# steinwurf/storage-benchmarks

Measured on AMD Instinct MI355X. Metric: encode+decode goodput GiB/s (device-resident) at symbols x symbol_size; %HBM roofline, higher is better.
Workload: dtype u8; 1 GPU; isa_throughput c3: symbols=64 symbol_size=1000000 loss_rate=0.5 erased=32 blocks_per_gpu=1024; symbols=64, symbol_size=1000000, erased=32, parallelism=blocks sharded x1, no collective, decode_kernel=auto, encode_kernel=auto

## Files before the change

storage-benchmarks_amd/csrc/jit_prog.cpp:

```cpp
#include "jit_prog.h"

#include <string.h>

#include <algorithm>

#include "rs_jit.h"
#include "rs_kernels.h"

namespace rsgpu {
namespace jit {

namespace {

inline int value_reg(int v, int bank) { return v < 8 ? plane_reg(bank, v) : 32 + (v - 8); }

void full_tables(const uint8_t (&masks)[8 * kMaxSlots], int nm, SrcProg& p)
{
    uint8_t id[256];
    memset(id, kNone, sizeof id);
    for (int a = 0; a < 8; ++a)
        id[1 << a] = (uint8_t)a;
    p.nops = 0;
    for (int hi = 0; hi < 2; ++hi)
        for (int n = 1; n < 16; ++n) {
// ... 505 lines not shown
            for (int b = 0; b < 8; ++b)
                acc[b] = 40 + 8 * r + b;
            if (!emit_scale_add(w, role == 1 ? 1 : kp.sigma[r], 10, 18, acc))
                return 0;
        }
        w.put64(ret);
        return w.o;
    }
    const uint8_t* m = role == 0 ? kp.cP : role == 1 ? kp.cQ1 : kp.cQ2;
    for (int i = 0; i < kKaraPairs; ++i) {
        const int s = kKaraPairs * ch + i;
        if (role == 0) {
            emit_load_planes(w, 10, 2 * i);
            emit_load_planes(w, 18, 2 * i + 1);
            w.put32(enc_waitcnt_lgkm(0));
            const int pl[8] = {10, 11, 12, 13, 14, 15, 16, 17};
            if (!emit_scale_add(w, kp.rho[s], 18, 26, pl))
                return 0;
        } else {
            emit_load_planes(w, 10, 2 * i + (role - 1));
            w.put32(enc_waitcnt_lgkm(0));
        }
        uint8_t cf[16];
        for (int r = 0; r < 16; ++r)
            cf[r] = m[r * 32 + s];
        SrcProg prog;
        plan_source(cf, 16, prog);
        emit_source_body(w, 16, prog);
    }
    w.put64(ret);
    return w.o;
}

}

bool build_karatsuba_code(const uint8_t* c, KaraProgram* out)
{
    KaraProgram& kp = *out;
    auto c2 = [](int n) { return n * (n - 1) / 2; };
    auto h = [&](int n) { return gf_pow2(c2(n)); };
    uint8_t d[64], D1[32];
    for (int j = 0; j < 64; ++j)
        d[j] = gf_pow2(-c2(j));
    for (int r = 0; r < 32; ++r)
        D1[r] = gf_pow2(-c2(r));
    for (int r = 0; r < 16; ++r)
        kp.sigma[r] = gf_mul(D1[r + 16], gf_inv(D1[r]));
    for (int base = 0; base < 64; base += 32)
        for (int q = 0; q < 16; ++q) {
            const int s = 16 * (base / 32) + q;
            kp.rho[s] = gf_mul(d[base + 16 + q], gf_inv(d[base + q]));
            for (int r = 0; r < 16; ++r) {
                const uint8_t hb = h(r + q + base + 16);
                kp.cP[r * 32 + s] = gf_mul(gf_mul(D1[r], hb), d[base + q]);
                kp.cQ1[r * 32 + s] = gf_mul(gf_mul(D1[r], (uint8_t)(h(r + q + base) ^ hb)), d[base + q]);
                kp.cQ2[r * 32 + s] =
                    gf_mul(gf_mul(D1[r + 16], (uint8_t)(h(r + q + base + 32) ^ hb)), d[base + 16 + q]);
                const uint8_t p = kp.cP[r * 32 + s], pr = gf_mul(p, kp.rho[s]);
                if ((uint8_t)(p ^ kp.cQ1[r * 32 + s]) != c[r * 64 + base + q] || pr != c[r * 64 + base + 16 + q] ||
                    gf_mul(kp.sigma[r], p) != c[(16 + r) * 64 + base + q] ||
                    (uint8_t)(gf_mul(kp.sigma[r], pr) ^ kp.cQ2[r * 32 + s]) != c[(16 + r) * 64 + base + 16 + q])
                    return false;
            }
        }
    size_t most = 0;
    for (int role = 0; role < 3; ++role)
        for (int ch = 0; ch < kKaraChunks; ++ch) {
            const size_t n = emit_chunk_kara(nullptr, kp, role, ch);
            if (!n)
                return false;
            most = std::max(most, n);
        }
    kp.chunk_stride = (int)((most + 63) / 64 * 64);
    kp.code.assign((size_t)3 * kKaraChunks * kp.chunk_stride, 0);
    for (size_t i = 0; i + 8 <= kp.code.size(); i += 8) {
        const uint64_t ret = (uint64_t)S_NOP0 << 32 | S_SETPC_82;
        memcpy(&kp.code[i], &ret, 8);
    }
    for (int role = 0; role < 3; ++role)
        for (int ch = 0; ch < kKaraChunks; ++ch)
            emit_chunk_kara(&kp.code[((size_t)role * kKaraChunks + ch) * kp.chunk_stride], kp, role, ch);
    return true;
}

}
}
```

storage-benchmarks_amd/csrc/jit_prog.h:

```cpp
#pragma once
#include <stddef.h>
#include <stdint.h>

#include <utility>
#include <vector>

namespace rsgpu {
namespace jit {

constexpr int kMaxComposites = 22;
constexpr uint8_t kNone = 255;

constexpr int kMaxSlots = 16;

struct SrcProg {
    int nops = 0;
    uint8_t ops[kMaxComposites][3];
    uint8_t outs[8 * kMaxSlots][2];
};

void plan_source(const uint8_t* coef, int nslot, SrcProg& p, int max_ops = kMaxComposites);

int host_chunk_stride();

size_t emit_chunk(uint8_t* dst, int nt, int nslot, const SrcProg* progs);

std::vector<uint8_t> build_matrix_code(const uint8_t* c, int k, int e, int* chunk_stride,
                                       int max_ops = kMaxComposites);

std::vector<uint8_t> build_matrix_code_wide(const uint8_t* c, int k, int e, int R, int CS, int* chunk_stride,
                                            int max_ops = kMaxComposites);

std::vector<uint8_t> build_matrix_code_wide_passes(const uint8_t* c, int k, int e,
                                                   std::vector<std::pair<size_t, int>>* passes,
                                                   int max_ops = kMaxComposites);

struct KaraProgram {
    std::vector<uint8_t> code;
    int chunk_stride = 0;
    uint8_t cP[16 * 32], cQ1[16 * 32], cQ2[16 * 32];
    uint8_t rho[32], sigma[16];
};

bool build_karatsuba_code(const uint8_t* c, KaraProgram* out);

}
}
```

storage-benchmarks_amd/csrc/rs_jit.h:

```cpp
#pragma once
#include <stdint.h>

#include "jit_enc.h"
#include "kernel_hooks.h"

namespace rsgpu {
namespace jit {

constexpr int ACC = 64;
constexpr int PRO_BYTES = 16;
constexpr int PRE_BYTES = 112;
constexpr int EPI_BYTES = 8;

RJ_HD constexpr int src_bytes(int nslot) { return PRE_BYTES + 64 * nslot; }
RJ_HD constexpr int chunk_bytes(int nt, int nslot) { return PRO_BYTES + nt * src_bytes(nslot) + EPI_BYTES; }
RJ_HD constexpr int chunk_stride(int nslot) { return (chunk_bytes(8, nslot) + 63) / 64 * 64; }

RJ_HD constexpr int plane_reg(int bank, int a) { return (bank ? 54 : 24) + a; }

RJ_HD constexpr int table_reg(int bank, int hi, int n)
{
    if ((n & (n - 1)) == 0) {
        const int a = n == 1 ? 0 : n == 2 ? 1 : n == 4 ? 2 : 3;
        return plane_reg(bank, 4 * hi + a);
// ... 138 lines not shown
        const int low = n & -n;
        return enc_xor_e32(treg(hi, n), treg(hi, n ^ low), treg(hi, low));
    }

    RJ_HD static bool code_word(const uint8_t* rows, int k, int nslot, int ch, int o, uint64_t* word)
    {
        const int nt = k - CS * ch < CS ? k - CS * ch : CS;
        const int per_src = PRE / 8 + 8 * nslot;
        if (o < nt * per_src) {
            const int t = o / per_src, r = o - t * per_src;
            if (r < PRE / 8) {
                *word = (uint64_t)pre_u32(t, 2 * r + 1) << 32 | pre_u32(t, 2 * r);
            } else {
                const int m = r - PRE / 8, s = m >> 3;
                uint64_t wd[8];
                mac_words(rows[s * k + CS * ch + t], s, wd);
                *word = wd[m & 7];
            }
        } else if (o == nt * per_src) {
            *word = (uint64_t)S_NOP0 << 32 | S_SETPC_82;
        } else {
            return false;
        }
        return true;
    }
};
using J16 = Wide<16, 6>;
using J12 = Wide<12, 6>;
using J10 = Wide<10, 5>;

constexpr int kKaraPairs = 4;
constexpr int kKaraSrcChunks = 32 / kKaraPairs;
constexpr int kKaraChunks = kKaraSrcChunks + 1;
RJ_HD constexpr int kara_source(int ch, int t)
{
    const int s = kKaraPairs * ch + t / 2;
    return 32 * (s / 16) + (s % 16) + 16 * (t & 1);
}

struct WideTables {
    static constexpr int PW = Wide<16, 6>::PRE / 8;
    uint64_t mac[256 * 8];
    uint64_t pre[6 * PW];
};
RJ_HD constexpr WideTables wide_tables()
{
    WideTables w{};
    for (int c = 0; c < 256; ++c)
        for (int b = 0; b < 8; ++b)
            w.mac[8 * c + b] = J16::mac_base(mat_row((uint8_t)c, b));
    for (int t = 0; t < 6; ++t)
        for (int r = 0; r < WideTables::PW; ++r)
            w.pre[WideTables::PW * t + r] = (uint64_t)J16::pre_u32(t, 2 * r + 1) << 32 | J16::pre_u32(t, 2 * r);
    return w;
}

}
}
```

storage-benchmarks_amd/csrc/rs_jit.hip:

```cpp
#include <hip/hip_runtime.h>
#include <stdint.h>

#include <algorithm>
#include <cstring>
#include <type_traits>
#include <utility>

#include "bitslice.h"
#include "diag_clock.h"
#include "rs_jit.h"
#include "rs_kernels.h"
#include "rs_lane.h"
#include "rs_span.h"
#include "tc_handlers.inc"

namespace rsgpu {
namespace jitk {

using bs::barrier_lds;
using bs::glds32;
using bs::glds32_nt;
using bs::sload_ptr;
using bs::store32;
using bs::tr8;
// ... 741 lines not shown
                         : RSGPU_JW_CALL_CLOBBERS, "s82", "s83", "scc", "memory", RSGPU_J12_ACC_CLOBBERS);
        else
            asm volatile("s_swappc_b64 s[82:83], %[fn]"
                         :
                         : [fn] "s"(fn), "{v9}"(la)
                         : RSGPU_JW_CALL_CLOBBERS, "s82", "s83", "scc", "memory", RSGPU_J10_ACC_CLOBBERS);
        ph.mark(5);
    }
    epi.template run<W, TPW, NV>(a, dsts, bw, wave, tw, lane, off, &lds[0][0][0]);
    ph.mark(6);
    ph.end(wv);
}

template <class W, int TPW, int NV>
__global__ __launch_bounds__(64 * NV * TPW) __attribute__((amdgpu_num_vgpr(40))) void k_rs_jitw(JitArgs a)
{
    __shared__ uint4 lds[2][TPW][W::CS * 2 * 64];
    RSGPU_DIAG_BEGIN()
    const int wv = __builtin_amdgcn_readfirstlane(threadIdx.x >> 6);
    const int wave = wv % NV, tw = wv / NV;
    const int lane = threadIdx.x & 63;
    RSGPU_JIT_PLACE(a, b, wg)
    const long long tile = wg * TPW + tw;
    if (a.status && a.status[b] != 0)
        return;
    jitw_run<W, TPW, NV>(a, lds, wv, wave, tw, lane, b, wg, tile, JitwStore{});
    RSGPU_DIAG_END();
}

__global__ __launch_bounds__(64 * 3) __attribute__((amdgpu_num_vgpr(40))) void k_rs_kara(JitArgs a)
{
    constexpr int CS = 2 * jit::kKaraPairs, NCH = jit::kKaraSrcChunks, K = 64;
    __shared__ uint4 lds[2][CS * 2 * 64];
    const int role = __builtin_amdgcn_readfirstlane(threadIdx.x >> 6);
    const int lane = threadIdx.x & 63;
    RSGPU_JIT_PLACE(a, b, tile)
    const uint8_t* const* srcs = a.srcs + (size_t)b * K;
    uint8_t* const* dsts = a.dsts + (size_t)b * a.dst_stride;
    const uint8_t* code = a.code + (size_t)role * jit::kKaraChunks * a.chunk_stride;
    const uint32_t lds0 = (uint32_t)(uintptr_t)(__attribute__((address_space(3))) uint4*)&lds[0][0];
    constexpr uint32_t kBuf = CS * 2 * 64 * 16;
    const long long off = tile * 2048 + lane * 32;
    const uint32_t loff = off + 32 <= a.len ? (uint32_t)off : 0u;
    if (role == 0)
        asm volatile("s_icache_inv\n s_nop 15\n s_nop 15" ::: "memory");
    typedef const uint8_t* const __attribute__((address_space(4)))* CPtrs;
    const CPtrs csrcs = (CPtrs)srcs;
    const int first = role == 0 ? 2 : role - 1;
    constexpr int PW = 3;
    auto ptrs = [&](int ch, const uint8_t* (&p)[PW]) {
#pragma unroll
        for (int i = 0; i < PW; ++i)
            p[i] = csrcs[jit::kara_source(ch, min(first + 3 * i, CS - 1))];
    };
    auto issue = [&](int par, const uint8_t* const (&p)[PW]) {
        const uint32_t base = lds0 + (uint32_t)(par * kBuf);
#pragma unroll
        for (int i = 0; i < PW; ++i) {
            const int t = first + 3 * i;
            if (t < CS)
                glds32(p[i], loff, base + (uint32_t)(t * 2 * 64 * 16));
        }
    };
    asm volatile(RSGPU_J16_ZERO ::: RSGPU_J16_ACC_CLOBBERS);
    int rot = 0;
    if (a.chunk_rot_ticks > 0) {
        volatile int& s_rot = *(volatile int*)&lds[1][0];
        if (threadIdx.x == 0) {
            unsigned long long t;
            asm volatile("s_memrealtime %0\n s_waitcnt lgkmcnt(0)" : "=s"(t)::"memory");
            const unsigned long long p = (unsigned long long)a.chunk_rot_ticks;
            s_rot = (int)(((t + p / 2) / p) % (unsigned long long)NCH);
        }
        __syncthreads();
        rot = __builtin_amdgcn_readfirstlane(s_rot);
    }
    auto chunk_of = [&](int i) { return i + rot >= NCH ? i + rot - NCH : i + rot; };
    const uint8_t* pc[PW];
    const uint8_t* pn[PW];
    ptrs(chunk_of(0), pc);
    issue(0, pc);
    ptrs(chunk_of(1), pn);
    for (int i = 0; i < NCH; ++i) {
        const int ch = chunk_of(i), par = i & 1;
        uint4* buf = lds[par];
        wait_vm(0);
        if (a.prio)
            asm volatile("s_setprio 2" ::: "memory");
        {
            const uint32_t m4 = vconst(0x0F0F0F0Fu), m2 = vconst(0x33333333u), m1 = vconst(0x55555555u);
            for (int t = first; t < CS; t += 3) {
                uint4 u = buf[(t * 2 + 0) * 64 + lane], v = buf[(t * 2 + 1) * 64 + lane];
                uint32_t Wd[8] = {u.x, u.y, u.z, u.w, v.x, v.y, v.z, v.w};
                tr8(Wd, m4, m2, m1);
                buf[(t * 2 + 0) * 64 + lane] = make_uint4(Wd[0], Wd[1], Wd[2], Wd[3]);
                buf[(t * 2 + 1) * 64 + lane] = make_uint4(Wd[4], Wd[5], Wd[6], Wd[7]);
            }
        }
        barrier_lds();
        if (a.prio)
            asm volatile("s_setprio 0" ::: "memory");
        if (i + 1 < NCH)
            issue(par ^ 1, pn);
        ptrs(chunk_of(min(i + 2, NCH - 1)), pn);
        const uint32_t la = lds0 + (uint32_t)(par * kBuf) + lane * 16;
        const uint8_t* fn = code + (size_t)ch * a.chunk_stride;
        asm volatile("s_swappc_b64 s[82:83], %[fn]"
                     :
                     : [fn] "s"(fn), "{v9}"(la)
                     : RSGPU_JW_CALL_CLOBBERS, "s82", "s83", "scc", "memory", RSGPU_J16_ACC_CLOBBERS);
    }
    barrier_lds();
    if (role == 0) {
        uint4* tb = &lds[0][0];
        [&]<int... Ss>(std::integer_sequence<int, Ss...>) {
            (
                [&] {
                    uint32_t Wd[8];
                    read_slotw<Ss>(Wd);
                    tb[(Ss * 2 + 0) * 64 + lane] = make_uint4(Wd[0], Wd[1], Wd[2], Wd[3]);
                    tb[(Ss * 2 + 1) * 64 + lane] = make_uint4(Wd[4], Wd[5], Wd[6], Wd[7]);
                }(),
                ...);
        }(std::make_integer_sequence<int, 16>{});
    }
    barrier_lds();
    if (role != 0) {
        const uint32_t la = lds0 + lane * 16;
        const uint8_t* fn = code + (size_t)NCH * a.chunk_stride;
        asm volatile("s_swappc_b64 s[82:83], %[fn]"
                     :
                     : [fn] "s"(fn), "{v9}"(la)
                     : RSGPU_JW_CALL_CLOBBERS, "s82", "s83", "scc", "memory", RSGPU_J16_ACC_CLOBBERS);
        const int half = role - 1;
        JitwStore{}.run<jit::J16, 1, 2>(a, dsts, b, half, 0, lane, off, nullptr);
    }
}

template <class W, int TPW, int NV>
__global__ __launch_bounds__(64 * NV * TPW) __attribute__((amdgpu_num_vgpr(40))) void k_rs_jitw_scrub(JitScrubArgs s)
{
    __shared__ uint4 lds[2][TPW][W::CS * 2 * 64];
    const int wv = __builtin_amdgcn_readfirstlane(threadIdx.x >> 6);
    const int wave = wv % NV, tw = wv / NV;
    const int lane = threadIdx.x & 63;
    RSGPU_JIT_PLACE(s.j, b, wg)
    const long long tile = wg * TPW + tw;
    jitw_run<W, TPW, NV>(s.j, lds, wv, wave, tw, lane, b, wg, tile, JitwScrub{{s.fold, s.tab, s.locate}});
}

template <class W, int TPW, int NV>
__global__ __launch_bounds__(64 * NV * TPW) __attribute__((amdgpu_num_vgpr(40))) void k_rs_jitw_locate(JitLocateArgs s)
{
    __shared__ uint4 lds[2][TPW][W::CS * 2 * 64];
    const int wv = __builtin_amdgcn_readfirstlane(threadIdx.x >> 6);
    const int wave = wv % NV, tw = wv / NV;
    const int lane = threadIdx.x & 63;
    RSGPU_JIT_PLACE(s.j, b, wg)
    const long long tile = wg * TPW + tw;
    jitw_run<W, TPW, NV>(s.j, lds, wv, wave, tw, lane, b, wg, tile,
                         JitwLocate{{s.fold, s.cand, s.cand_stride, s.slots, s.u}});
}

template <class W, int TPW, int NV>
__global__ __launch_bounds__(64 * NV * TPW) __attribute__((amdgpu_num_vgpr(40))) void k_rs_jitw_repair(JitRepairArgs s)
{
    __shared__ uint4 lds[2][TPW][W::CS * 2 * 64];
    const int wv = __builtin_amdgcn_readfirstlane(threadIdx.x >> 6);
    const int wave = wv % NV, tw = wv / NV;
// ... 420 lines not shown
```

storage-benchmarks_amd/csrc/rs_kernels.h:

```cpp
#pragma once
#include <hip/hip_runtime.h>
#include <stdint.h>

struct rsgpu_scrub_report;

namespace rsgpu {

constexpr size_t kMaxGridBlocks = 65535;

struct DotArgs {
    const uint8_t* const* srcs;
    uint8_t* const* dsts;
    const uint4* tabs4;
    const uint32_t* ctab;
    long long tab_block_stride;
    int k, rows, rows_pad;
    long long len;
    long long blocks;
    const int* status;
    bool bytewise;
};

struct PrepArgs {
    int k, m, nerrs, rows_pad;
// ... 82 lines not shown
    long long pitch, len, blocks;
    int k, e;
    const uint8_t* rowtab;
    const uint8_t* coef;
    RepairFold* fold;
    int mode;
};
hipError_t launch_repair_compare(const RepairCmpArgs& a, hipStream_t st);
hipError_t launch_repair_finalise(void* report, long long blocks, int mode, hipStream_t st);
hipError_t launch_rs_bitsliced_repair(int k, int e, uint8_t* src, uint8_t* par, long long pitch, long long len,
                                      long long blocks, RepairFold* fold, int mode, hipStream_t st);

hipError_t launch_decode_prepare_syn(int k, int e, long long blocks, const uint8_t* err,
                                     uint8_t* out, long long out_pitch, const uint8_t** srcs,
                                     uint8_t** dsts, const unsigned long long* tc_table, int* status,
                                     const uint8_t* src, const uint8_t* par,
                                     unsigned long long* dir_addr, uint8_t* jit_coef, hipStream_t st);

struct JitArgs {
    const uint8_t* const* srcs;
    uint8_t* const* dsts;
    const uint8_t* code;
    long long chunk_stride;
    long long block_stride;
    int k, rows;
    int dst_stride;
    long long len;
    const int* status;
    int xcd_order;
    int tiles_per_wg = 1;
    int code_prefetch = 0;
    int chunk_rot_ticks = 0;
    int prio = 0;
};
int jitw_rot_ticks(int rows);
size_t jit_code_bytes(int k, int e, long long blocks);
hipError_t launch_jit_emit(int k, int e, long long blocks, const uint8_t* coef, const int* status,
                           uint8_t* code, hipStream_t st);
hipError_t launch_jit_fill(void* code, size_t bytes, hipStream_t st);
hipError_t launch_rs_jit(const JitArgs& a, long long blocks, hipStream_t st);
int jitw_rows(int e);
int jitw_cs(int e);
size_t jitw_chunk_stride(int e);
size_t jitw_code_bytes(int k, int e, long long blocks);
bool jitw_layout(int e);
size_t jitw_pass_bytes(int k, int rows);
size_t jitw_pass_offset(int k, int e, int p);
hipError_t launch_jitw_emit(int k, int e, long long blocks, const uint8_t* coef, const int* status,
                            uint8_t* code, hipStream_t st);
hipError_t launch_rs_jitw(const JitArgs& a, long long blocks, hipStream_t st);
hipError_t launch_rs_kara(const JitArgs& a, long long blocks, hipStream_t st);
struct JitScrubArgs {
    JitArgs j;
    ScrubFold* fold;
    const uint8_t* tab;
    int locate;
};
hipError_t launch_rs_jit_scrub(const JitScrubArgs& a, long long blocks, hipStream_t st);
struct JitLocateArgs {
    JitArgs j;
    ScrubFold* fold;
    uint8_t* cand;
    size_t cand_stride;
    int slots;
    int u;
};
// ... 207 lines not shown
```

storage-benchmarks_amd/csrc/rsgpu_capi.cpp:

```cpp
#include <hip/hip_runtime.h>
#include <hsa/hsa.h>
#include <hsa/hsa_ext_amd.h>

#include <algorithm>
#include <climits>
#include <cstdio>
#include <cstdlib>
#include <cstring>
#include <string>
#include <vector>

#include "../../include/rsgpu.h"
#include "gf256.h"
#include "rsgpu_ctx.h"
#include "rsgpu_internal.h"
#include "jit_prog.h"
#include "rs_jit.h"
#include "rs_kernels.h"
#include "rs_synth.h"

namespace {

using namespace rsgpu;

// ... 47 lines not shown
    hsa_amd_memory_pool_get_info(p, HSA_AMD_MEMORY_POOL_INFO_RUNTIME_ALLOC_ALLOWED, &alloc);
    if ((flags & HSA_AMD_MEMORY_POOL_GLOBAL_FLAG_COARSE_GRAINED) && alloc) {
        *(hsa_amd_memory_pool_t*)out = p;
        return HSA_STATUS_INFO_BREAK;
    }
    return HSA_STATUS_SUCCESS;
}

constexpr size_t kProgCacheEntries = 64;
constexpr size_t kProgCacheBytes = 256u << 20;

const rsgpu_ctx::SharedProg* shared_program(rsgpu_ctx* ctx, const uint8_t* coef, int k, int rows, int* rc_out,
                                            bool kara = false)
{
    *rc_out = RSGPU_OK;
    const bool wide = jitw_layout(rows);
    std::vector<uint8_t> key(9 + (size_t)k * rows);
    std::memcpy(key.data(), &k, 4);
    std::memcpy(key.data() + 4, &rows, 4);
    key[8] = kara ? 2 : wide ? 1 : 0;
    std::memcpy(key.data() + 9, coef, (size_t)k * rows);
    for (auto& pr : ctx->progs)
        if (pr.key == key) {
            pr.last = ++ctx->prog_tick;
            return &pr;
        }
    auto err = [&](int code, const char* msg) -> const rsgpu_ctx::SharedProg* {
        *rc_out = fail(ctx, code, msg);
        return nullptr;
    };
    if (jit_probe(ctx) != 1)
        return err(RSGPU_ERR_UNSUPPORTED, "no executable device memory pool");
    int stride = 0;
    std::vector<uint8_t> code;
    std::vector<std::pair<size_t, int>> passes;
    if (kara) {
        jit::KaraProgram kp;
        if (k != 64 || rows != 32 || !jit::build_karatsuba_code(coef, &kp))
            return err(RSGPU_ERR_UNSUPPORTED, "Karatsuba program: not the (64, 32) gf_gen_rs_matrix code");
        code = std::move(kp.code);
        stride = kp.chunk_stride;
    } else if (wide) {
        code = jit::build_matrix_code_wide_passes(coef, k, rows, &passes);
        if (code.empty())
            return err(RSGPU_ERR_UNSUPPORTED, "shared program: rows exceed the layout");
    } else {
        code = jit::build_matrix_code(coef, k, rows, &stride);
    }
    size_t used = 0;
    for (const auto& pr : ctx->progs)
        used += pr.bytes;
    if (!ctx->progs.empty() &&
        (ctx->progs.size() >= kProgCacheEntries || used + code.size() > kProgCacheBytes)) {
        if (hipStreamSynchronize(ctx->stream) != hipSuccess)
            return err(RSGPU_ERR_HIP, "shared program: draining the stream before an eviction");
        while (!ctx->progs.empty() &&
               (ctx->progs.size() >= kProgCacheEntries || used + code.size() > kProgCacheBytes)) {
            auto lru = std::min_element(ctx->progs.begin(), ctx->progs.end(),
                                        [](const auto& a, const auto& b) { return a.last < b.last; });
            used -= lru->bytes;
            hsa_amd_memory_pool_free(lru->code);
            ctx->progs.erase(lru);
        }
    }
    if (ctx->code_stage_bytes < code.size()) {
        if (hipStreamSynchronize(ctx->stream) != hipSuccess)
            return err(RSGPU_ERR_HIP, "shared program: draining the stream before regrowing the stage");
        if (ctx->d_code_stage)
            (void)hipFree(ctx->d_code_stage);
        ctx->d_code_stage = nullptr;
        ctx->code_stage_bytes = 0;
        if (hipMalloc(&ctx->d_code_stage, code.size()) != hipSuccess)
            return err(RSGPU_ERR_NOMEM, "shared program: code stage allocation failed");
        ctx->code_stage_bytes = code.size();
    }
    rsgpu_ctx::SharedProg pr;
    if (hsa_amd_memory_pool_allocate(ctx->jit_pool, code.size(), HSA_AMD_MEMORY_POOL_EXECUTABLE_FLAG,
                                     &pr.code) != HSA_STATUS_SUCCESS || !pr.code)
        return err(RSGPU_ERR_NOMEM, "executable device allocation failed");
    pr.bytes = code.size();
    void* stage;
    int rc = get_stage(ctx, code.size(), &stage);
    if (!rc) {
        std::memcpy(stage, code.data(), code.size());
        rc = upload(ctx, ctx->d_code_stage, code.size());
    }
    if (!rc && launch_jit_copy(pr.code, ctx->d_code_stage, code.size(), ctx->stream) != hipSuccess)
        rc = fail(ctx, RSGPU_ERR_HIP, "shared program: copy into executable memory");
    if (rc) {
        hsa_amd_memory_pool_free(pr.code);
        *rc_out = rc;
        return nullptr;
    }
    pr.key = std::move(key);
    pr.chunk_stride = stride;
    pr.passes = std::move(passes);
    pr.last = ++ctx->prog_tick;
    ctx->progs.push_back(std::move(pr));
    return &ctx->progs.back();
}

JitArgs shared_pass_args(const rsgpu_ctx* ctx, const rsgpu_ctx::SharedProg* pg, int k, int rows, int p,
                         long long len, const uint8_t* const* d_srcs, uint8_t* const* d_dsts)
{
    if (jitw_layout(rows)) {
        JitArgs j = jit_args(d_srcs, d_dsts + jit::wide_pass_row0(rows, p),
                             (const uint8_t*)pg->code + pg->passes[p].first, pg->passes[p].second, 0, k,
                             jit::wide_pass_rows(rows, p), rows, len, nullptr);
        j.tiles_per_wg = ctx->jitw_tpw ? ctx->jitw_tpw : 2;
        j.chunk_rot_ticks = ctx->jitw_rot >= 0 ? ctx->jitw_rot : jitw_rot_ticks(j.rows);
        j.prio = ctx->jitw_prio;
        return j;
    }
    const int nch = (k + 7) / 8;
    JitArgs j = jit_args(d_srcs, d_dsts + 32 * p, (const uint8_t*)pg->code + (size_t)p * 4 * nch * pg->chunk_stride,
                         pg->chunk_stride, 0, k, std::min(32, rows - 32 * p), rows, len, nullptr);
    j.prio = 0;
    return j;
}

int shared_program_launch(rsgpu_ctx* ctx, const uint8_t* coef, int k, int rows, long long len,
                          long long blocks, const uint8_t* const* d_srcs, uint8_t* const* d_dsts,
                          const char* name)
{
    int rc = RSGPU_OK;
    const rsgpu_ctx::SharedProg* pg = shared_program(ctx, coef, k, rows, &rc);
    if (!pg)
        return rc;
    const bool wide = jitw_layout(rows);
    for (int p = 0; wide ? p < jit::wide_passes(rows) : p * 32 < rows; ++p) {
// ... 98 lines not shown
size_t dot_table_bytes(int k, int rows)
{
    return std::max(sizeof(unsigned long long) * (size_t)tc_table_elems(k, rows),
                    (size_t)k * rows_pad_for(rows) * (sizeof(uint4) + sizeof(uint32_t)));
}

constexpr long long kKaraMinWork = 480000;
constexpr int kKaraRotTicks = 400;

int karatsuba_launch(rsgpu_ctx* ctx, long long len, size_t pitch, size_t blocks, const unsigned char* d_src,
                     unsigned char* d_parity, bool* unavailable)
{
    const int k = 64, e = 32;
    *unavailable = false;
    const std::vector<uint8_t> c = parity_matrix(k, e, nullptr);
    int rc = RSGPU_OK;
    const std::string err_before = ctx->err;
    const rsgpu_ctx::SharedProg* pg = shared_program(ctx, c.data(), k, e, &rc, true);
    if (!pg && rc == RSGPU_ERR_UNSUPPORTED) {
        ctx->kara_state = -1;
        ctx->err = err_before;
        *unavailable = true;
        return RSGPU_OK;
    }
    if (!pg)
        return rc;
    RowPtrs rp;
    rc = row_ptr_tables(ctx, k, e, pitch, blocks, d_src, d_parity, rp);
    if (rc)
        return rc;
    JitArgs j = jit_args(rp.src, rp.par, pg->code, pg->chunk_stride, 0, k, e, e, len, nullptr);
    j.chunk_rot_ticks = ctx->jitw_rot >= 0 ? ctx->jitw_rot : kKaraRotTicks;
    j.prio = ctx->jitw_prio;
    KTimer kt(ctx, "k_rs_jit(encode)", blocks);
    RS_HIP(ctx, launch_rs_kara(j, (long long)blocks, ctx->stream));
    return RSGPU_OK;
}

int encode_slice(rsgpu_ctx* ctx, int k, int e, size_t len, size_t pitch, size_t blocks, const unsigned char* d_src,
                 unsigned char* d_parity, const unsigned char* coef)
{
    const bool aligned = ptrs_aligned(pitch, d_src, d_parity);
    const bool kara_wanted = ctx->encode_kernel == RSGPU_ENCODE_KARATSUBA ||
                             (ctx->encode_kernel == RSGPU_ENCODE_AUTO &&
                              (long long)(tiles(len) * blocks) >=
                                  (ctx->kara_min_work >= 0 ? ctx->kara_min_work : kKaraMinWork));
    if (kara_wanted && ctx->kara_state >= 0 && !coef && k == 64 && e == 32 && aligned && len % 32 == 0 &&
        jit_probe(ctx) == 1) {
        bool unavailable;
        const int rc = karatsuba_launch(ctx, (long long)len, pitch, blocks, d_src, d_parity, &unavailable);
        if (!unavailable)
            return rc;
    }
    const bool compiled_ok = ctx->encode_kernel == RSGPU_ENCODE_AUTO || ctx->encode_kernel == RSGPU_ENCODE_COMPILED ||
                             ctx->encode_kernel == RSGPU_ENCODE_KARATSUBA;
    if (compiled_ok && !coef && aligned && len % 32 == 0 && rs_bitsliced_split_available(k, e) &&
        (long long)(tiles(len) * blocks) < kTcSplitMaxWork) {
        KTimer kt(ctx, "k_rs_bs_split(encode)", blocks);
        RS_HIP(ctx, launch_rs_bitsliced_split(k, e, d_src, d_parity, (long long)pitch, (long long)len,
                                              (long long)blocks, ctx->stream));
        return RSGPU_OK;
    }
    const bool compiled_pays = ctx->encode_kernel == RSGPU_ENCODE_COMPILED ||
                               rs_bitsliced_rows_per_wave(k, e) >= 8 || !jitw_rows(e) ||
                               !(len % 32 == 0 && jit_probe(ctx) == 1);
    if (compiled_ok && compiled_pays && !coef && aligned && len % 32 == 0 && rs_bitsliced_available(k, e)) {
// ... 255 lines not shown
    return RSGPU_OK;
}

int rsgpu_destroy(rsgpu_ctx* ctx)
{
    if (!ctx)
        return RSGPU_ERR_ARG;
    (void)hipSetDevice(ctx->device);
    (void)hipStreamSynchronize(ctx->stream);
    for (void* p : {ctx->scratch.p, ctx->scrub.p, ctx->d_update, ctx->degraded.p, ctx->rebuild.p,
                    ctx->locate.p})
        if (p)
            (void)hipFree(p);
    if (ctx->h_stage)
        (void)hipHostFree(ctx->h_stage);
    if (ctx->stage_done)
        (void)hipEventDestroy(ctx->stage_done);
    for (auto& r : ctx->recs) {
        (void)hipEventDestroy(r.a);
        (void)hipEventDestroy(r.b);
    }
    for (auto e : ctx->ev_pool)
        (void)hipEventDestroy(e);
    for (auto e : ctx->sync_evs)
        (void)hipEventDestroy(e);
    if (ctx->d_tc_table)
        (void)hipFree(ctx->d_tc_table);
    if (ctx->d_jit)
        hsa_amd_memory_pool_free(ctx->d_jit);
    for (auto& pr : ctx->progs)
        hsa_amd_memory_pool_free(pr.code);
    if (ctx->d_code_stage)
        (void)hipFree(ctx->d_code_stage);
    for (hipStream_t st : {ctx->io_in, ctx->io_out, ctx->aux})
        if (st) {
            (void)hipStreamSynchronize(st);
            (void)hipStreamDestroy(st);
        }
    if (ctx->d_io)
        (void)hipFree(ctx->d_io);
    for (auto e : ctx->io_evs)
        (void)hipEventDestroy(e);
    delete ctx;
    return RSGPU_OK;
}

int rsgpu_set_stream(rsgpu_ctx* ctx, void* s)
{
    if (!ctx)
        return RSGPU_ERR_ARG;
    hipStream_t ns = (hipStream_t)s;
    if (ns == ctx->stream)
        return RSGPU_OK;
    hipEvent_t ev = sync_event(ctx);
    hipError_t e = hipEventRecord(ev, ctx->stream);
    if (e == hipSuccess)
        e = hipStreamWaitEvent(ns, ev, 0);
    ctx->stream = ns;
    if (e != hipSuccess)
        return fail(ctx, RSGPU_ERR_HIP, std::string("rsgpu_set_stream: ordering against the old stream: ") +
                                            hipGetErrorString(e));
    return RSGPU_OK;
}

void* rsgpu_get_stream(rsgpu_ctx* ctx) { return ctx ? (void*)ctx->stream : nullptr; }

// ... 316 lines not shown
```

storage-benchmarks_amd/csrc/rsgpu_ctx.h:

```cpp
#pragma once
#include <hip/hip_runtime.h>
#include <hsa/hsa.h>
#include <hsa/hsa_ext_amd.h>

#include <string>
#include <vector>

#include "../../include/rsgpu.h"

struct rsgpu_ctx {
    int device = 0;
    hipStream_t stream = nullptr;
    std::vector<hipEvent_t> sync_evs;
    size_t sync_next = 0;
    unsigned long long* d_tc_table = nullptr;
    unsigned long long h_tc_table[2048] = {};
    unsigned long long tc_base = 0;
    int tc_state = 0;
    int decode_kernel = RSGPU_DECODE_AUTO;
    int jitw_tpw = 0;
    long long kara_min_work = -1;
    int kara_state = 0;
    int jitw_prefetch = -1;
    int jitw_rot = -1;
    int bs_prio = 2;
    int jitw_prio = 2;
    int decode_pipe = -1;
    hipStream_t aux = nullptr;
    void* d_jit = nullptr;
    size_t jit_bytes = 0;
    int jit_state = 0;
    unsigned long long jit_gen = 0;
    struct {
        int k = 0, e = 0;
        size_t blocks = 0;
        const void* ws = nullptr;
        unsigned long long gen = 0;
    } jit_key;
    hsa_amd_memory_pool_t jit_pool{};
    int encode_kernel = RSGPU_ENCODE_AUTO;
    struct SharedProg {
        std::vector<uint8_t> key;
        void* code = nullptr;
        size_t bytes = 0;
        int chunk_stride = 0;
        std::vector<std::pair<size_t, int>> passes;
        unsigned long long last = 0;
    };
    std::vector<SharedProg> progs;
    unsigned long long prog_tick = 0;
    void* d_code_stage = nullptr;
    size_t code_stage_bytes = 0;
    std::string err;
    struct DevBuf {
        void* p = nullptr;
        size_t bytes = 0;
        std::vector<uint8_t> key;
    };
    DevBuf scratch;
    int scrub_kernel = RSGPU_SCRUB_AUTO;
    DevBuf scrub;
    void* d_update = nullptr;
    std::vector<uint8_t> update_key;
    DevBuf degraded;
    int degraded_kernel = RSGPU_DEGRADED_AUTO;
    int correct_kernel = RSGPU_CORRECT_AUTO;
    int repair_kernel = RSGPU_REPAIR_KERNEL_AUTO;
    DevBuf rebuild;
    int rebuild_kernel = RSGPU_REBUILD_AUTO;
    struct RebuildWideLayout {
        size_t blocks = 0, lane = 0, lane_stride = 0, addr = 0, srcs = 0, dsts = 0, count = 0;
        int k = 0, passes = 0, slots = 0;
    } rebuild_wide;
    size_t rebuild_group_max = 0;
    bool rebuild_prepare_only = false;
    int locate_kernel = RSGPU_LOCATE_AUTO;
    DevBuf locate;
    size_t locate_group_max = 0;
    void* h_stage = nullptr;
    size_t stage_bytes = 0;
    hipEvent_t stage_done = nullptr;
    bool stage_pending = false;
    bool timing = false;
// ... 47 lines not shown
```

storage-benchmarks_amd/csrc/rsgpu_testhooks.cpp:

```cpp
#include <hip/hip_runtime.h>

#include <algorithm>
#include <cstdint>
#include <cstring>
#include <vector>

#include "../../include/rsgpu.h"
#include "jit_prog.h"
#include "plane_mul.h"
#include "rs_jit.h"
#include "rs_kernels.h"
#include "rs_lane.h"
#include "rs_pairs.h"
#include "rsgpu_ctx.h"

using namespace rsgpu;

namespace {

template <class W>
void jitw_emit_host(int k, int row_base, int rows, const unsigned char* coef, uint64_t* o64)
{
    const int nch = (k + W::CS - 1) / W::CS, stride_w = W::chunk_stride() / 8;
    for (int w = 0; w < jit::wide_waves(rows); ++w) {
// ... 185 lines not shown
                                          size_t out_bytes, long long* pass_off, int* pass_stride, int max_passes,
                                          int* npasses, int max_ops)
{
    if (k <= 0 || k + e > 250 || !jitw_layout(e) || !coef || !pass_off || !pass_stride || !npasses)
        return -1;
    std::vector<std::pair<size_t, int>> passes;
    const std::vector<uint8_t> code = jit::build_matrix_code_wide_passes(coef, k, e, &passes, max_ops);
    if (code.empty() || (int)passes.size() > max_passes)
        return -1;
    *npasses = (int)passes.size();
    for (size_t p = 0; p < passes.size(); ++p) {
        pass_off[p] = (long long)passes[p].first;
        pass_stride[p] = passes[p].second;
    }
    if (out && out_bytes >= code.size())
        std::memcpy(out, code.data(), code.size());
    return (long long)code.size();
}

long long rsgpu_internal_jit_karatsuba_code(const unsigned char* coef, unsigned char* out, size_t out_bytes,
                                            int* chunk_stride, unsigned char* mats)
{
    jit::KaraProgram kp;
    if (!coef || !chunk_stride || !jit::build_karatsuba_code(coef, &kp))
        return -1;
    *chunk_stride = kp.chunk_stride;
    if (mats) {
        std::memcpy(mats, kp.cP, 512);
        std::memcpy(mats + 512, kp.cQ1, 512);
        std::memcpy(mats + 1024, kp.cQ2, 512);
        std::memcpy(mats + 1536, kp.rho, 32);
        std::memcpy(mats + 1568, kp.sigma, 16);
    }
    if (out && out_bytes >= kp.code.size())
        std::memcpy(out, kp.code.data(), kp.code.size());
    return (long long)kp.code.size();
}

int rsgpu_internal_set_kara_min_work(rsgpu_ctx* ctx, long long pairs)
{
    if (!ctx || pairs < -1)
        return RSGPU_ERR_ARG;
    ctx->kara_min_work = pairs;
    return RSGPU_OK;
}

int rsgpu_internal_set_kara_state(rsgpu_ctx* ctx, int state)
{
    if (!ctx || (state != 0 && state != -1))
        return RSGPU_ERR_ARG;
    ctx->kara_state = state;
    return RSGPU_OK;
}

long long rsgpu_internal_jitw_emit_device(rsgpu_ctx* ctx, int k, int e, size_t blocks,
                                          const unsigned char* coef, unsigned char* out, size_t out_bytes)
{
    if (!ctx || k <= 0 || !jitw_layout(e) || k + e > 250 || blocks == 0 || blocks > kMaxGridBlocks || !coef)
        return -1;
    const size_t need = jitw_code_bytes(k, e, (long long)blocks);
    if (!out || out_bytes < need)
        return (long long)need;
    uint8_t *d_coef = nullptr, *d_code = nullptr;
    int* d_status = nullptr;
    long long rc = -1;
    if (hipMalloc(&d_coef, blocks * e * k) == hipSuccess && hipMalloc(&d_code, need) == hipSuccess &&
        hipMalloc(&d_status, blocks * sizeof(int)) == hipSuccess &&
        hipMemcpyAsync(d_coef, coef, blocks * e * k, hipMemcpyHostToDevice, ctx->stream) == hipSuccess &&
        hipMemsetAsync(d_status, 0, blocks * sizeof(int), ctx->stream) == hipSuccess &&
        launch_jit_fill(d_code, need, ctx->stream) == hipSuccess &&
        launch_jitw_emit(k, e, (long long)blocks, d_coef, d_status, d_code, ctx->stream) == hipSuccess &&
        hipMemcpyAsync(out, d_code, need, hipMemcpyDeviceToHost, ctx->stream) == hipSuccess &&
        hipStreamSynchronize(ctx->stream) == hipSuccess)
        rc = (long long)need;
    (void)hipFree(d_coef);
    (void)hipFree(d_code);
// ... 68 lines not shown
```

Baseline: 1443 GiB/s.

## Split Karatsuba epilogue across three waves and gate icache invalidation by generation

The Karatsuba encode kernel's final combine step, previously done by two waves while wave 0 only staged slots, is now split so all three waves run JIT-emitted epilogue chunks and each stores part of the parity rows directly. Separately, the per-launch s_icache_inv is replaced by a per-CU generation table, so the cache is invalidated only when a newer code upload is seen. This aims to balance epilogue work across waves and to avoid repeated instruction-cache flushes. In exchange it adds an extra LDS barrier round, a global atomic table, and a dependency on hardware-ID registers for per-CU slot indexing.

```diff
diff --git a/storage-benchmarks_amd/csrc/jit_prog.cpp b/storage-benchmarks_amd/csrc/jit_prog.cpp
--- a/storage-benchmarks_amd/csrc/jit_prog.cpp
+++ b/storage-benchmarks_amd/csrc/jit_prog.cpp
@@ -561,6 +561,42 @@
     return w.o;
 }
 
+size_t emit_chunk_kara_epi(uint8_t* dst, const KaraProgram& kp, int role, int round)
+{
+    Writer w{dst};
+    auto slot = [](int s, int (&acc)[8]) {
+        for (int b = 0; b < 8; ++b)
+            acc[b] = 40 + 8 * s + b;
+    };
+    int acc[8];
+    if (role == 0 && round == 0) {
+        for (int r = 0; r < kKaraSplit; ++r) {
+            emit_load_planes(w, 10, 8 + r);
+            w.put32(enc_waitcnt_lgkm(0));
+            for (int b = 0; b < 8; ++b)
+                w.put64(enc_xor_e64(40 + 8 * (8 + r) + b, 40 + 8 * r + b, 10 + b));
+        }
+        for (int r = 0; r < kKaraSplit; ++r) {
+            slot(12 + r, acc);
+            emit_load_planes(w, acc[0], 12 + r);
+            w.put32(enc_waitcnt_lgkm(0));
+            if (!emit_scale_add(w, kp.sigma[r], 40 + 8 * r, 10, acc))
+                return 0;
+        }
+    } else if (role != 0) {
+        const int n = round == 0 ? 8 : kKaraSplit, row0 = round == 0 ? 8 : kKaraSplit, pos0 = round == 0 ? 0 : 8;
+        for (int r = 0; r < n; ++r) {
+            emit_load_planes(w, 10, pos0 + r);
+            w.put32(enc_waitcnt_lgkm(0));
+            slot(row0 + r, acc);
+            if (!emit_scale_add(w, role == 1 ? 1 : kp.sigma[row0 + r], 10, 18, acc))
+                return 0;
+        }
+    }
+    w.put64((uint64_t)S_NOP0 << 32 | S_SETPC_82);
+    return w.o;
+}
+
 }
 
 bool build_karatsuba_code(const uint8_t* c, KaraProgram* out)
@@ -600,8 +636,16 @@
                 return false;
             most = std::max(most, n);
         }
+    for (int role = 0; role < 3; ++role)
+        for (int round = 0; round < kKaraEpiChunks; ++round) {
+            const size_t n = emit_chunk_kara_epi(nullptr, kp, role, round);
+            if (!n)
+                return false;
+            most = std::max(most, n);
+        }
     kp.chunk_stride = (int)((most + 63) / 64 * 64);
-    kp.code.assign((size_t)3 * kKaraChunks * kp.chunk_stride, 0);
+    kp.epi_offset = (size_t)3 * kKaraChunks * kp.chunk_stride;
+    kp.code.assign(kp.epi_offset + (size_t)3 * kKaraEpiChunks * kp.chunk_stride, 0);
     for (size_t i = 0; i + 8 <= kp.code.size(); i += 8) {
         const uint64_t ret = (uint64_t)S_NOP0 << 32 | S_SETPC_82;
         memcpy(&kp.code[i], &ret, 8);
@@ -609,6 +653,10 @@
     for (int role = 0; role < 3; ++role)
         for (int ch = 0; ch < kKaraChunks; ++ch)
             emit_chunk_kara(&kp.code[((size_t)role * kKaraChunks + ch) * kp.chunk_stride], kp, role, ch);
+    for (int role = 0; role < 3; ++role)
+        for (int round = 0; round < kKaraEpiChunks; ++round)
+            emit_chunk_kara_epi(&kp.code[kp.epi_offset + ((size_t)role * kKaraEpiChunks + round) * kp.chunk_stride], kp,
+                                role, round);
     return true;
 }
 
diff --git a/storage-benchmarks_amd/csrc/jit_prog.h b/storage-benchmarks_amd/csrc/jit_prog.h
--- a/storage-benchmarks_amd/csrc/jit_prog.h
+++ b/storage-benchmarks_amd/csrc/jit_prog.h
@@ -38,6 +38,7 @@
 struct KaraProgram {
     std::vector<uint8_t> code;
     int chunk_stride = 0;
+    size_t epi_offset = 0;
     uint8_t cP[16 * 32], cQ1[16 * 32], cQ2[16 * 32];
     uint8_t rho[32], sigma[16];
 };
diff --git a/storage-benchmarks_amd/csrc/rs_jit.h b/storage-benchmarks_amd/csrc/rs_jit.h
--- a/storage-benchmarks_amd/csrc/rs_jit.h
+++ b/storage-benchmarks_amd/csrc/rs_jit.h
@@ -194,6 +194,9 @@
 constexpr int kKaraPairs = 4;
 constexpr int kKaraSrcChunks = 32 / kKaraPairs;
 constexpr int kKaraChunks = kKaraSrcChunks + 1;
+constexpr int kKaraEpiChunks = 2;
+constexpr int kKaraSplit = 4;
+constexpr int kIcacheGenSlots = 16 * 256;
 RJ_HD constexpr int kara_source(int ch, int t)
 {
     const int s = kKaraPairs * ch + t / 2;
diff --git a/storage-benchmarks_amd/csrc/rs_jit.hip b/storage-benchmarks_amd/csrc/rs_jit.hip
--- a/storage-benchmarks_amd/csrc/rs_jit.hip
+++ b/storage-benchmarks_amd/csrc/rs_jit.hip
@@ -797,6 +797,7 @@
 {
     constexpr int CS = 2 * jit::kKaraPairs, NCH = jit::kKaraSrcChunks, K = 64;
     __shared__ uint4 lds[2][CS * 2 * 64];
+    JitwPhases ph;
     const int role = __builtin_amdgcn_readfirstlane(threadIdx.x >> 6);
     const int lane = threadIdx.x & 63;
     RSGPU_JIT_PLACE(a, b, tile)
@@ -807,8 +808,19 @@
     constexpr uint32_t kBuf = CS * 2 * 64 * 16;
     const long long off = tile * 2048 + lane * 32;
     const uint32_t loff = off + 32 <= a.len ? (uint32_t)off : 0u;
-    if (role == 0)
-        asm volatile("s_icache_inv\n s_nop 15\n s_nop 15" ::: "memory");
+    unsigned* gen_slot = nullptr;
+    unsigned gen_seen = 0;
+    if (role == 0) {
+        if (a.icache_gen) {
+            unsigned x, h;
+            asm volatile("s_getreg_b32 %0, hwreg(HW_REG_XCC_ID)\n s_getreg_b32 %1, hwreg(HW_REG_HW_ID)"
+                         : "=s"(x), "=s"(h));
+            gen_slot = a.icache_gen + (((x & 15u) << 8) | ((h >> 8) & 255u));
+            gen_seen = __hip_atomic_load(gen_slot, __ATOMIC_RELAXED, __HIP_MEMORY_SCOPE_AGENT);
+        } else {
+            asm volatile("s_icache_inv\n s_nop 15\n s_nop 15" ::: "memory");
+        }
+    }
     typedef const uint8_t* const __attribute__((address_space(4)))* CPtrs;
     const CPtrs csrcs = (CPtrs)srcs;
     const int first = role == 0 ? 2 : role - 1;
@@ -846,10 +858,17 @@
     ptrs(chunk_of(0), pc);
     issue(0, pc);
     ptrs(chunk_of(1), pn);
+    if (gen_slot && (unsigned)__builtin_amdgcn_readfirstlane((int)gen_seen) < a.code_gen) {
+        asm volatile("s_icache_inv\n s_nop 15\n s_nop 15" ::: "memory");
+        if (lane == 0)
+            __hip_atomic_store(gen_slot, a.code_gen, __ATOMIC_RELAXED, __HIP_MEMORY_SCOPE_AGENT);
+    }
     for (int i = 0; i < NCH; ++i) {
         const int ch = chunk_of(i), par = i & 1;
         uint4* buf = lds[par];
+        ph.mark(0);
         wait_vm(0);
+        ph.mark(1);
         if (a.prio)
             asm volatile("s_setprio 2" ::: "memory");
         {
@@ -862,44 +881,105 @@
                 buf[(t * 2 + 1) * 64 + lane] = make_uint4(Wd[4], Wd[5], Wd[6], Wd[7]);
             }
         }
+        ph.mark(2);
         barrier_lds();
+        ph.mark(3);
         if (a.prio)
             asm volatile("s_setprio 0" ::: "memory");
         if (i + 1 < NCH)
             issue(par ^ 1, pn);
         ptrs(chunk_of(min(i + 2, NCH - 1)), pn);
+        ph.mark(4);
         const uint32_t la = lds0 + (uint32_t)(par * kBuf) + lane * 16;
         const uint8_t* fn = code + (size_t)ch * a.chunk_stride;
         asm volatile("s_swappc_b64 s[82:83], %[fn]"
                      :
                      : [fn] "s"(fn), "{v9}"(la)
                      : RSGPU_JW_CALL_CLOBBERS, "s82", "s83", "scc", "memory", RSGPU_J16_ACC_CLOBBERS);
+        ph.mark(5);
     }
     barrier_lds();
-    if (role == 0) {
-        uint4* tb = &lds[0][0];
-        [&]<int... Ss>(std::integer_sequence<int, Ss...>) {
-            (
-                [&] {
-                    uint32_t Wd[8];
-                    read_slotw<Ss>(Wd);
-                    tb[(Ss * 2 + 0) * 64 + lane] = make_uint4(Wd[0], Wd[1], Wd[2], Wd[3]);
-                    tb[(Ss * 2 + 1) * 64 + lane] = make_uint4(Wd[4], Wd[5], Wd[6], Wd[7]);
-                }(),
-                ...);
-        }(std::make_integer_sequence<int, 16>{});
-    }
-    barrier_lds();
-    if (role != 0) {
+    uint4* tb = &lds[0][0];
+    auto row_off = [&] {
+        int l = lane;
+        asm volatile("" : "+v"(l));
+        return tile * 2048 + l * 32;
+    };
+    auto put_slots = [&]<int S0, int P0, int... Is>(std::integer_sequence<int, S0, P0, Is...>) {
+        (
+            [&] {
+                uint32_t Wd[8];
+                read_slotw<S0 + Is>(Wd);
+                tb[((P0 + Is) * 2 + 0) * 64 + lane] = make_uint4(Wd[0], Wd[1], Wd[2], Wd[3]);
+                tb[((P0 + Is) * 2 + 1) * 64 + lane] = make_uint4(Wd[4], Wd[5], Wd[6], Wd[7]);
+            }(),
+            ...);
+    };
+    auto call = [&](const uint8_t* fn) {
         const uint32_t la = lds0 + lane * 16;
-        const uint8_t* fn = code + (size_t)NCH * a.chunk_stride;
         asm volatile("s_swappc_b64 s[82:83], %[fn]"
                      :
                      : [fn] "s"(fn), "{v9}"(la)
                      : RSGPU_JW_CALL_CLOBBERS, "s82", "s83", "scc", "memory", RSGPU_J16_ACC_CLOBBERS);
-        const int half = role - 1;
-        JitwStore{}.run<jit::J16, 1, 2>(a, dsts, b, half, 0, lane, off, nullptr);
-    }
+    };
+    if (!a.epi_code) {
+        if (role == 0)
+            put_slots(std::integer_sequence<int, 0, 0, 0, 1, 2, 3, 4, 5, 6, 7, 8, 9, 10, 11, 12, 13, 14, 15>{});
+        barrier_lds();
+        if (role != 0) {
+            call(code + (size_t)NCH * a.chunk_stride);
+            ph.mark(6);
+            const int half = role - 1;
+            const long long off_e = row_off();
+            JitwStore{}.run<jit::J16, 1, 2>(a, dsts, b, half, 0, lane, off_e, nullptr);
+        } else {
+            ph.mark(6);
+        }
+        ph.end(role);
+        return;
+    }
+    constexpr int M = jit::kKaraSplit;
+    static_assert(M == 4, "the slot lists below are written for a split of 4 rows");
+    const uint8_t* epi = a.epi_code + (size_t)role * jit::kKaraEpiChunks * a.chunk_stride;
+    if (role == 0)
+        put_slots(std::integer_sequence<int, 8, 0, 0, 1, 2, 3, 4, 5, 6, 7>{});
+    else if (role == 1)
+        put_slots(std::integer_sequence<int, 0, 8, 0, 1, 2, 3>{});
+    else
+        put_slots(std::integer_sequence<int, 0, 12, 0, 1, 2, 3>{});
+    barrier_lds();
+    call(epi);
+    if (role == 0)
+        put_slots(std::integer_sequence<int, 4, 8, 0, 1, 2, 3>{});
+    barrier_lds();
+    if (role != 0)
+        call(epi + a.chunk_stride);
+    ph.mark(6);
+    typedef uint8_t* const __attribute__((address_space(4)))* CDsts;
+    const long long off_e = row_off();
+    const bool live = off_e + 32 <= a.len;
+    auto store_slots = [&]<int S0, int... Is>(int row0, std::integer_sequence<int, S0, Is...>) {
+        uint8_t* dp[sizeof...(Is)];
+        ((dp[Is] = ((CDsts)dsts)[row0 + Is]), ...);
+        if (live) {
+            const uint32_t m4 = vconst(0x0F0F0F0Fu), m2 = vconst(0x33333333u), m1 = vconst(0x55555555u);
+            (
+                [&] {
+                    uint32_t Wd[8];
+                    read_slotw<S0 + Is>(Wd);
+                    tr8(Wd, m4, m2, m1);
+                    store32(dp[Is], off_e, Wd);
+                }(),
+                ...);
+        }
+    };
+    if (role == 0) {
+        store_slots(0, std::integer_sequence<int, 8, 0, 1, 2, 3>{});
+        store_slots(16, std::integer_sequence<int, 12, 0, 1, 2, 3>{});
+    } else {
+        store_slots(16 * (role - 1) + M, std::integer_sequence<int, 4, 0, 1, 2, 3, 4, 5, 6, 7, 8, 9, 10, 11>{});
+    }
+    ph.end(role);
 }
 
 template <class W, int TPW, int NV>
diff --git a/storage-benchmarks_amd/csrc/rs_kernels.h b/storage-benchmarks_amd/csrc/rs_kernels.h
--- a/storage-benchmarks_amd/csrc/rs_kernels.h
+++ b/storage-benchmarks_amd/csrc/rs_kernels.h
@@ -138,6 +138,9 @@
     int code_prefetch = 0;
     int chunk_rot_ticks = 0;
     int prio = 0;
+    unsigned* icache_gen = nullptr;
+    unsigned code_gen = 0;
+    const uint8_t* epi_code = nullptr;
 };
 int jitw_rot_ticks(int rows);
 size_t jit_code_bytes(int k, int e, long long blocks);
diff --git a/storage-benchmarks_amd/csrc/rsgpu_capi.cpp b/storage-benchmarks_amd/csrc/rsgpu_capi.cpp
--- a/storage-benchmarks_amd/csrc/rsgpu_capi.cpp
+++ b/storage-benchmarks_amd/csrc/rsgpu_capi.cpp
@@ -103,6 +103,7 @@
     if (jit_probe(ctx) != 1)
         return err(RSGPU_ERR_UNSUPPORTED, "no executable device memory pool");
     int stride = 0;
+    size_t epi_offset = 0;
     std::vector<uint8_t> code;
     std::vector<std::pair<size_t, int>> passes;
     if (kara) {
@@ -111,6 +112,7 @@
             return err(RSGPU_ERR_UNSUPPORTED, "Karatsuba program: not the (64, 32) gf_gen_rs_matrix code");
         code = std::move(kp.code);
         stride = kp.chunk_stride;
+        epi_offset = kp.epi_offset;
     } else if (wide) {
         code = jit::build_matrix_code_wide_passes(coef, k, rows, &passes);
         if (code.empty())
@@ -167,6 +169,8 @@
     pr.chunk_stride = stride;
     pr.passes = std::move(passes);
     pr.last = ++ctx->prog_tick;
+    pr.gen = ++ctx->code_gen;
+    pr.epi_offset = epi_offset;
     ctx->progs.push_back(std::move(pr));
     return &ctx->progs.back();
 }
@@ -331,6 +335,22 @@
     JitArgs j = jit_args(rp.src, rp.par, pg->code, pg->chunk_stride, 0, k, e, e, len, nullptr);
     j.chunk_rot_ticks = ctx->jitw_rot >= 0 ? ctx->jitw_rot : kKaraRotTicks;
     j.prio = ctx->jitw_prio;
+    if (ctx->kara_epilogue)
+        j.epi_code = (const uint8_t*)pg->code + pg->epi_offset;
+    if (ctx->kara_inv) {
+        if (!ctx->d_icache_gen) {
+            const size_t bytes = jit::kIcacheGenSlots * sizeof(unsigned);
+            if (hipMalloc(&ctx->d_icache_gen, bytes) != hipSuccess)
+                return fail(ctx, RSGPU_ERR_NOMEM, "Karatsuba encode: instruction-cache generation table");
+            if (hipMemsetAsync(ctx->d_icache_gen, 0, bytes, ctx->stream) != hipSuccess) {
+                (void)hipFree(ctx->d_icache_gen);
+                ctx->d_icache_gen = nullptr;
+                return fail(ctx, RSGPU_ERR_HIP, "Karatsuba encode: zeroing the generation table");
+            }
+        }
+        j.icache_gen = ctx->d_icache_gen;
+        j.code_gen = pg->gen;
+    }
     KTimer kt(ctx, "k_rs_jit(encode)", blocks);
     RS_HIP(ctx, launch_rs_kara(j, (long long)blocks, ctx->stream));
     return RSGPU_OK;
@@ -652,6 +672,8 @@
         hsa_amd_memory_pool_free(pr.code);
     if (ctx->d_code_stage)
         (void)hipFree(ctx->d_code_stage);
+    if (ctx->d_icache_gen)
+        (void)hipFree(ctx->d_icache_gen);
     for (hipStream_t st : {ctx->io_in, ctx->io_out, ctx->aux})
         if (st) {
             (void)hipStreamSynchronize(st);
diff --git a/storage-benchmarks_amd/csrc/rsgpu_ctx.h b/storage-benchmarks_amd/csrc/rsgpu_ctx.h
--- a/storage-benchmarks_amd/csrc/rsgpu_ctx.h
+++ b/storage-benchmarks_amd/csrc/rsgpu_ctx.h
@@ -46,9 +46,15 @@
         int chunk_stride = 0;
         std::vector<std::pair<size_t, int>> passes;
         unsigned long long last = 0;
+        unsigned gen = 0;
+        size_t epi_offset = 0;
     };
     std::vector<SharedProg> progs;
     unsigned long long prog_tick = 0;
+    unsigned code_gen = 0;
+    unsigned* d_icache_gen = nullptr;
+    int kara_inv = 1;
+    int kara_epilogue = 1;
     void* d_code_stage = nullptr;
     size_t code_stage_bytes = 0;
     std::string err;
diff --git a/storage-benchmarks_amd/csrc/rsgpu_testhooks.cpp b/storage-benchmarks_amd/csrc/rsgpu_testhooks.cpp
--- a/storage-benchmarks_amd/csrc/rsgpu_testhooks.cpp
+++ b/storage-benchmarks_amd/csrc/rsgpu_testhooks.cpp
@@ -241,9 +241,30 @@
         std::memcpy(mats + 1536, kp.rho, 32);
         std::memcpy(mats + 1568, kp.sigma, 16);
     }
-    if (out && out_bytes >= kp.code.size())
-        std::memcpy(out, kp.code.data(), kp.code.size());
-    return (long long)kp.code.size();
+    if (out && out_bytes >= kp.epi_offset)
+        std::memcpy(out, kp.code.data(), kp.epi_offset);
+    return (long long)kp.epi_offset;
+}
+
+long long rsgpu_internal_jit_karatsuba_epilogue_code(const unsigned char* coef, unsigned char* out, size_t out_bytes,
+                                                     int* chunk_stride)
+{
+    jit::KaraProgram kp;
+    if (!coef || !chunk_stride || !jit::build_karatsuba_code(coef, &kp))
+        return -1;
+    *chunk_stride = kp.chunk_stride;
+    const size_t n = kp.code.size() - kp.epi_offset;
+    if (out && out_bytes >= n)
+        std::memcpy(out, kp.code.data() + kp.epi_offset, n);
+    return (long long)n;
+}
+
+int rsgpu_internal_set_kara_epilogue(rsgpu_ctx* ctx, int three_way)
+{
+    if (!ctx || (three_way != 0 && three_way != 1))
+        return RSGPU_ERR_ARG;
+    ctx->kara_epilogue = three_way;
+    return RSGPU_OK;
 }
 
 int rsgpu_internal_set_kara_min_work(rsgpu_ctx* ctx, long long pairs)
@@ -251,6 +272,14 @@
     if (!ctx || pairs < -1)
         return RSGPU_ERR_ARG;
     ctx->kara_min_work = pairs;
+    return RSGPU_OK;
+}
+
+int rsgpu_internal_set_kara_inv(rsgpu_ctx* ctx, int per_upload)
+{
+    if (!ctx || (per_upload != 0 && per_upload != 1))
+        return RSGPU_ERR_ARG;
+    ctx->kara_inv = per_upload;
     return RSGPU_OK;
 }
 
```

Result: no change. 1446 GiB/s, median of 6 (+0.2%).
